# fritzsedlazeck/Sniffles

Hardware: AMD Instinct MI355X
Metric: SV-signatures clustered/sec (clustering + calling + QC + genotype + INS consensus) (higher is better)
Workload: dtype int32/f64

## Files before the change

### sniffles_amd/csrc/snf_fused.h

```cpp
#pragma once
#include "snf_stage_final.h"
#include "snf_stage_cluster.h"
#include "snf_stage_call.h"

namespace snf {

template <int K>
SNF_D void block_exscan256(const unsigned long long (&val)[K], unsigned long long (&excl)[K], unsigned long long (&tot)[K],
                           unsigned long long* lds) {
  const int tid = threadIdx.x, lane = tid & 63, wid = tid >> 6;
  unsigned long long incl[K];
#pragma unroll
  for (int k = 0; k < K; k++) {
    unsigned long long x = val[k];
#pragma unroll
    for (int d = 1; d < 64; d <<= 1) { const unsigned long long y = __shfl_up(x, d, 64); if (lane >= d) x += y; }
    incl[k] = x;
    if (lane == 63) lds[wid * K + k] = x;
  }
  __syncthreads();
#pragma unroll
  for (int k = 0; k < K; k++) {
    unsigned long long base = 0, all = 0;
#pragma unroll
// ... 93 lines not shown
          }
        }
        const unsigned long long inc = __ballot(state == 2);
        const int first = __ffsll((long long)inc) - 1;
        unsigned long long part = (inc == 0 || lane <= first) ? w : 0ull;
#pragma unroll
        for (int d = 32; d >= 1; d >>= 1) part += __shfl_xor(part, d, 64);
        ex += part;
        if (inc) done = true; else j -= 64;
      }
      if (lane == 0) { st_agent_u64(&st[2 * tile + 1], tagI | (ex + tot[k])); lds[k] = ex; }
    }
  }
  __syncthreads();
#pragma unroll
  for (int k = 0; k < K; k++) { off[k] = lds[k] + excl[k]; total[k] = lds[k] + tot[k]; }
  __syncthreads();
}
#define SNF_CHAIN_HEAD(name, slot)                                            \
  __global__ void __launch_bounds__(256) name(const View v, int64_t n) {      \
    __shared__ unsigned long long lds[24];                                    \
    const int64_t tile = chain_ticket(v, slot, lds);                          \
    const int64_t p = tile * 256 + threadIdx.x;


#define SNF_FUSED_HEAD(name)                                                  \
  __global__ void __launch_bounds__(256) name(const View v, int64_t n) {      \
    __shared__ unsigned long long lds[8];                                     \
    const int64_t p = (int64_t)blockIdx.x * 256 + threadIdx.x;

__global__ void __launch_bounds__(256) z0_init(const View v, int64_t n) {
  const int64_t i = (int64_t)blockIdx.x * 256 + threadIdx.x;
  const int64_t T = v.T, G = 8 * T + 8;
  if (i < (int64_t)(sizeof(Counts) / 8)) ((unsigned long long*)v.cnt)[i] = 0;
  if (i <= T) { v.t_cov_sum[i] = 0; v.t_status[i] = 0; }
  if (i <= T + 1) v.t_call_off[i] = 0;
  if (i < G) { v.grp_first_bin[i] = -1; v.grp_seed_lo[i] = -1; v.grp_seed_hi[i] = -1; v.grp_dirty[i] = 0; }
  if (i < TS_SLOTS * v.super_stride) v.tile_super[i] = 0;
  if (i < v.tile_stride) {
    v.tile_sums[(int64_t)TS_REFINED * v.tile_stride + i] = 0; v.tile_sums[(int64_t)TS_CALLS * v.tile_stride + i] = 0;
  }
  if (i == 0) *v.chain_epoch += 1u;
  if (v.wave_path && i < 3 * 64 * 16) v.big_cnt[i] = 0;
  if (v.wave_path && i < 3 * 64 * 16) v.d2cnt[i] = 0;
  if (i == 0 && v.NS > 0) {
    const int64_t N = v.NS;
    v.headflag[N] = 0; v.eligflag[N] = 0; v.fN[N] = 0; v.fL[N] = 0; v.runflag[N] = 0; v.clflag[N] = 0; v.rcflag[N] = 0; v.cdflag[N] = 0;
  }
}

SNF_FUSED_HEAD(a0k_keep)
  if (p < n) a0_keep_body(p, v);
  unsigned long long val[1] = {p < n ? (unsigned long long)v.pf_keep[p] : 0ull};
  tile_publish<1>(v, TS_KEEP, val, lds);
}
SNF_FUSED_HEAD(a0k_compact)
  unsigned long long val[1] = {p < n ? (unsigned long long)v.pf_keep[p] : 0ull}, off[1];
  tile_scan<1>(v, TS_KEEP, val, off, lds);
  if (p < n) {
    v.pf_scan[p] = (uint32_t)off[0];
    if (p == n - 1) v.cnt->n_kept = (int64_t)(off[0] + val[0]);
    a0_emit(p, v);
  }
}
SNF_FUSED_HEAD(a2k_heads)
  if (p < n) { a2_heads_body(p, v); v.rcflag[p] = 0; }
  unsigned long long val[1] = {p < n ? (unsigned long long)v.headflag[p] : 0ull};
// ... 201 lines not shown
```

### sniffles_amd/csrc/snf_lib.hip

```cpp
#include "snf_stage_final.h"
#include "snf_wave_refine.h"
#include "snf_wave_cons.h"
#include "snf_fused.h"
#include "snf_stage_window.h"
#include "snf_stage_out.h"
#include "snf_wave_call.h"
#include "snf_wave_call_g.h"
#include "snf_wave_refine_g.h"
#include "snf_ctx.h"

#include <rocprim/device/device_radix_sort.hpp>
#include <rocprim/device/device_scan.hpp>

#include <fcntl.h>
#include <sys/file.h>
#include <unistd.h>

#include <atomic>
#include <map>
#include <tuple>
#include <cmath>
#include <ctime>
#include <memory>
#include <mutex>
// ... 608 lines not shown
    so[i] = sl >= 0 ? t.seq_off[i] + p0 : 0;
  }
}
void stage_pool(const snf_task_input_t& t, uint8_t* st, size_t pool_at, int64_t p0, int64_t b0, int64_t b1, std::atomic<int>* has_dash) {
  if (memchr(t.seq_pool + b0, '-', (size_t)(b1 - b0))) has_dash->store(1);
  memcpy(st + pool_at + (size_t)(p0 + b0), t.seq_pool + b0, (size_t)(b1 - b0));
}
void stage_reads(const snf_task_input_t& t, uint8_t* st, const size_t* off, int64_t r0, int32_t* rend_max) {
  const int64_t r = t.n_reads;
  int32_t* rs = (int32_t*)(st + off[IC_RSTART]) + r0; int32_t* re = (int32_t*)(st + off[IC_REND]) + r0;
  uint8_t* rh = st + off[IC_RHP] + r0;
  bool sorted = true;
  for (int64_t i = 1; i < r; i++) if (t.read_start[i] < t.read_start[i - 1]) { sorted = false; break; }
  if (sorted) {
    if (r) { memcpy(rs, t.read_start, (size_t)r * 4); memcpy(re, t.read_end, (size_t)r * 4); memcpy(rh, t.read_hp, (size_t)r); }
  } else {
    std::vector<int64_t> ord((size_t)r);
    for (int64_t i = 0; i < r; i++) ord[(size_t)i] = i;
    std::stable_sort(ord.begin(), ord.end(), [&](int64_t x, int64_t y) { return t.read_start[x] < t.read_start[y]; });
    for (int64_t i = 0; i < r; i++) { const int64_t k = ord[(size_t)i]; rs[i] = t.read_start[k]; re[i] = t.read_end[k]; rh[i] = t.read_hp[k]; }
  }
  int32_t rmax = 0;
  for (int64_t i = 0; i < r; i++) {
    const int32_t s = rs[i], e = re[i];
    if (s < 0 || s >= t.contig_len || e < s) fail("read interval outside the task region (leadprov.py:497-498)");
    if (rh[i] > 2) fail("read hp must be 0, 1 or 2");
    if (e > rmax) rmax = e;
  }
  *rend_max = rmax;
}

void enqueue_read_index(snf_batch_impl* b);
void enqueue_pass_init(snf_batch_impl* b);
void join_open_candidates(snf_batch_impl* b);
void enqueue_keys(snf_batch_impl* b);
bool coverage_per_call(const snf_batch_impl* b) { return b->k.d4_thread || !b->v.wave_path; }

void do_upload(snf_batch_impl* b) {
  SNF_TRACE("snf_batch_upload");
  View& v = b->v;
  const double t_begin = now_ms();
  int T = (int)b->tasks.size();
  int64_t N = b->h_lead_off.back(), R = b->h_read_off.back(), NTR = (int64_t)b->h_trs.size();
  if (T >= (1 << 16)) fail("too many tasks in one batch (max 65535)");
  if (N >= (int64_t)1 << 31 || R >= (int64_t)1 << 31) fail("batch too large for 32-bit lead/read indices");
  v.cfg = b->cfg; v.T = T; v.N = N; v.R = R; v.NTR = NTR;
  const int gap_base = b->cfg.cluster_merge_bnd > (int)b->cfg.cluster_repeat_h_max ? b->cfg.cluster_merge_bnd : (int)b->cfg.cluster_repeat_h_max;
  v.run_gap = b->k.run_gap != KNOB_UNSET ? b->k.run_gap : (gap_base > 1000 ? gap_base : 1000);
  v.wave_path = b->k.wave_path ? 1 : 0;
  b->fused = b->k.fuse && N <= ((int64_t)1 << 25);
  v.prof = b->k.prof ? 1 : 0;
  v.merge_reread = b->k.merge_reread ? 1 : 0;
  {
    int64_t max_bins = 1;
    for (auto& t : b->tasks) { int64_t nb = t.contig_len / (b->cfg.cluster_binsize > 0 ? b->cfg.cluster_binsize : 1) + 1; if (nb > max_bins) max_bins = nb; }
    v.key_bin_bits = bits_for((uint64_t)max_bins);
    v.key_nbits = v.key_bin_bits + bits_for((uint64_t)(8 * (T > 0 ? T : 1)));
    v.key32 = (!b->k.sort64 && v.key_nbits + 1 <= 32) ? 1 : 0;
  }
  v.pool_len = b->h_pool_off.back(); v.pool_cap = 2 * v.pool_len + 16;
  v.pool_extra_base = v.pool_len; v.pool_slice = 0;
  if (b->slots_d1w > 0 && b->k.pool_slices) {
    v.pool_slice = (v.pool_len / b->slots_d1w) & ~(int64_t)15;
    v.pool_extra_base = v.pool_len + v.pool_slice * b->slots_d1w;
    v.pool_cap = v.pool_extra_base + v.pool_len + 16;
  }
// ... 172 lines not shown
  size_t N1 = (size_t)N + 1;
  v.key_in = dalloc<uint64_t>(b, N); v.key_out = dalloc<uint64_t>(b, N); v.val_in = dalloc<uint32_t>(b, N); v.val_out = dalloc<uint32_t>(b, N);
  {
    v.NS = N; v.prefilter = 0;
    std::vector<int64_t> cell_off((size_t)T + 1, 0);
    const int bs = b->cfg.cluster_binsize > 0 ? b->cfg.cluster_binsize : 1;
    for (int t = 0; t < T; t++) cell_off[(size_t)t + 1] = cell_off[(size_t)t] + (int64_t)SNF_NTYPES * ((int64_t)b->tasks[(size_t)t].contig_len / bs + 1);
    const int64_t cells = cell_off[(size_t)T];
    if (N > 0 && b->cfg.dev_min_leads_cluster >= 2 && b->k.prefilter && cells < ((int64_t)1 << 36)) {
      v.prefilter = 1;
      v.t_cell_off = upload_vec(b, cell_off);
      b->pf_words = (((cells >> 19) + 1) << 19) / 16 + 2;
      v.pf_spread = b->k.pf_spread ? 1 : 0;
      v.pf_bm = dalloc<uint32_t>(b, (size_t)b->pf_words);
      dzero(b, v.pf_bm, (size_t)b->pf_words * 4);
      v.pf_key = dalloc<uint64_t>(b, N); v.pf_keep = dalloc<uint32_t>(b, N1); v.pf_scan = dalloc<uint32_t>(b, N1);
      dsync(b);
    }
  }
  const int WIN_W_MAX = b->k.win_bits_max, WIN_W_MIN = 6;
  auto win_layout = [&](int W, std::vector<int64_t>& off) {
    const int bs = b->cfg.cluster_binsize > 0 ? b->cfg.cluster_binsize : 1;
    off.assign((size_t)T + 1, 0);
    for (int t = 0; t < T; t++) off[(size_t)t + 1] = off[(size_t)t] + (int64_t)SNF_NTYPES * ((((int64_t)b->tasks[(size_t)t].contig_len / bs + 1) >> W) + 1);
    return off[(size_t)T];
  };
  int64_t win_slots_max = 0;
  const bool front_wanted = v.prefilter && v.wave_path && b->k.winfront && b->k.fuse && N <= ((int64_t)1 << 25) && T < (1 << 17);
  if (front_wanted) {
    std::vector<int64_t> off;
    win_slots_max = win_layout(WIN_W_MIN, off);
    if (win_slots_max >= ((int64_t)1 << 31)) win_slots_max = 0;
  }
  v.front = 0; v.NW = 0;
  if (win_slots_max > 0) {
    const size_t W1 = (size_t)win_slots_max + 1;
    v.wcnt = dalloc<uint32_t>(b, W1); v.wfill = dalloc<uint32_t>(b, W1); v.wbase = dalloc<uint32_t>(b, W1);
    const size_t occ_max = (size_t)(N < win_slots_max ? N : win_slots_max) + 2;
    const size_t nblk = (size_t)N / 64 + 2;
    v.wlist = dalloc<uint32_t>(b, 4 * occ_max); v.blk_k0 = dalloc<uint32_t>(b, nblk);
    v.ws_seeds = dalloc<uint32_t>(b, nblk); v.ws_nf = dalloc<uint32_t>(b, nblk); v.ws_nl = dalloc<uint32_t>(b, nblk);
    v.whead = dalloc<uint64_t>(b, N1); v.whead2 = dalloc<uint64_t>(b, N1);
    dzero(b, v.wcnt, W1 * 4); dzero(b, v.wfill, W1 * 4);
  }
  uint32_t** u32s[] = {&v.headflag, &v.headscan, &v.eligflag, &v.eligscan, &v.fN, &v.pN, &v.fL, &v.pL, &v.runflag, &v.runscan,
                       &v.clflag, &v.clscan, &v.rcflag, &v.rcscan, &v.cdflag, &v.cdscan, &v.rnf, &v.rnp};
  for (auto pp : u32s) *pp = dalloc<uint32_t>(b, N1);
  v.seqnull = dalloc<uint8_t>(b, N); v.bin_lo = dalloc<int32_t>(b, N1); v.bin_key = dalloc<uint64_t>(b, N);
  v.bin_hap = dalloc<uint16_t>(b, 3 * (size_t)N); v.bin_elig = dalloc<uint8_t>(b, N);
  v.grp_first_bin = dalloc<int32_t>(b, 8 * (size_t)T + 8);
  v.L = dalloc<uint32_t>(b, N); v.LL = dalloc<uint32_t>(b, N); v.Lrec = dalloc<LeadRec>(b, N1); v.chdr = dalloc<ClusterHdr>(b, N1);
  int32_t** i32s[] = {&v.seed_bin, &v.seed_lo, &v.seed_hi, &v.seedL_lo, &v.seedL_hi, &v.seed_start, &v.seed_grp, &v.c_last, &v.c_end,
                      &v.nxt, &v.prv, &v.run_first, &v.run_last_head, &v.cl_head, &v.w0, &v.w1, &v.w2, &v.w3, &v.w4, &v.w5, &v.w6, &v.w7,
                      &v.F_orig, &v.F_svlen, &v.F_seq_len, &v.FI, &v.F_lpos, &v.rc_n_s, &v.rc_cl_s, &v.rc_lo, &v.rc_n, &v.rc_cluster};
  for (auto pp : i32s) *pp = dalloc<int32_t>(b, N1);
  double** f64s[] = {&v.s_mean0, &v.s_stdev0, &v.c_mean, &v.c_stdev, &v.run_b_stdev, &v.run_b_absmean};
  for (auto pp : f64s) *pp = dalloc<double>(b, N1);
  uint8_t** u8s[] = {&v.s_repeat0, &v.c_repeat, &v.run_b_repeat, &v.F_sel, &v.rc_keeplong_s, &v.rc_keeplong};
  for (auto pp : u8s) *pp = dalloc<uint8_t>(b, N1);
  v.c_ms = dalloc<ClusterSums>(b, N1);
  v.grp_dirty = dalloc<int32_t>(b, 8 * (size_t)T + 8); v.grp_seed_lo = dalloc<int32_t>(b, 8 * (size_t)T + 8);
  v.grp_seed_hi = dalloc<int32_t>(b, 8 * (size_t)T + 8);
  v.F_seq_off = dalloc<int64_t>(b, N1);
  v.fcopy = dalloc<FuseDesc>(b, N1); dzero(b, v.fcopy, N1 * sizeof(FuseDesc));
  v.cand = dalloc<snf_call_t>(b, N1); v.candx = dalloc<CallX>(b, N1);
  v.calls = dalloc<snf_call_t>(b, N1); v.callx = dalloc<CallX>(b, N1);
  v.rnames = dalloc<uint32_t>(b, 2 * (size_t)N + 1);
// ... 18 lines not shown
  { const int eb = b->k.e1_batch; v.e1_batch = (eb == 2 || eb == 4 || eb == 8 || eb == 16 || eb == 32) ? eb : 64; }
  v.stage_cap = b->k.big_stage ? 1 : 0;
  v.cdesc = dalloc<ConsDesc>(b, N1); v.crl_off = dalloc<int64_t>(b, N1); v.crl_len = dalloc<int32_t>(b, N1); v.aln_kept_w = dalloc<uint8_t>(b, N1);
  for (int k = 0; k < 8; k++) v.cls_list[k] = k == 6 ? nullptr : dalloc<int32_t>(b, N1);
  v.d2cap = (int64_t)(N1 / 64 + 64);
  for (int k = 0; k < 3; k++) v.d2_list[k] = dalloc<int32_t>(b, (size_t)(64 * v.d2cap));
  v.d2cnt = dalloc<uint32_t>(b, 3 * 64 * 16);
  v.d2_from_list = 0; v.d1_from_list = 0;
#ifdef SNF_ITRACE
  if (!v.itrace) { SNF_HIP(hipMalloc((void**)&v.itrace, (size_t)SNF_IT_SLOTS * SNF_IT_CAP * 8)); SNF_HIP(hipMemset(v.itrace, 0, (size_t)SNF_IT_SLOTS * SNF_IT_CAP * 8)); }
#endif
#ifdef SNF_WG_TRACE
  if (!v.wgtrace) { SNF_HIP(hipMalloc((void**)&v.wgtrace, (size_t)(1 << 20) * 24)); SNF_HIP(hipMemset(v.wgtrace, 0, (size_t)(1 << 20) * 24)); }
#endif
  v.cons_tab_off = dalloc<int64_t>(b, N1 + 1); v.cons_aln_off = dalloc<int64_t>(b, N1 + 1); v.cons_read_off = dalloc<int64_t>(b, N1 + 1);
  v.cons_tab_sz = dalloc<int64_t>(b, N1 + 1);
  v.sz_tab = dalloc<int64_t>(b, N1 + 1); v.sz_aln = dalloc<int64_t>(b, N1 + 1); v.sz_rd = dalloc<int64_t>(b, N1 + 1);
  v.sc_tab = dalloc<int64_t>(b, N1 + 1); v.sc_aln = dalloc<int64_t>(b, N1 + 1); v.sc_rd = dalloc<int64_t>(b, N1 + 1);
  const double t_alloc = now_ms();
  if (v.prefilter) {
    const bool tm = b->timing; b->timing = false;
    enqueue_pass_init(b);
    enqueue_keys(b);
    b->timing = tm;
    Counts hc{};
    d2h(b, &hc, v.cnt, sizeof(Counts));
    dsync(b);
    v.NS = hc.n_kept;
    if (v.prof) fprintf(stderr, "[SNF_PROF] prefilter: %lld of %lld leads share their (svtype, bin) cell with another lead\n", (long long)v.NS, (long long)N);
  }
  const double t_pfcount = now_ms();
  if (win_slots_max > 0 && v.NS > 0) {
    int forced = b->k.win_bits;
    int best_w = -1; int64_t best_occ = 0, best_max = 0, best_big = 0;
    std::vector<int64_t> off;
    if (forced && (forced < WIN_W_MIN || forced > WIN_W_MAX)) forced = 0;
    for (int W = forced ? forced : WIN_W_MAX; W >= (forced ? forced : WIN_W_MIN); W--) {
      v.NW = win_layout(W, off); v.win_bits = W;
      const int64_t* d_off = upload_vec(b, off);
      v.t_win_off = d_off;
      const bool tm = b->timing; b->timing = false;
      enqueue_pass_init(b);
      LAUNCH_Q(w1_hist, v, N, 0);
      LAUNCH_Q(w0_stats, v, v.NW, 0);
      b->timing = tm;
      Counts hc{};
      d2h(b, &hc, v.cnt, sizeof(Counts));
      dzero(b, v.wcnt, ((size_t)v.NW + 1) * 4);
      dsync(b);
      if (hc.max_win <= 256 || (best_w < 0 && hc.max_win <= SNF_WIN_MAXCAP)) { best_w = W; best_occ = hc.n_occ; best_max = hc.max_win; best_big = hc.n_big64; }
      if (hc.max_win <= 256) break;
    }
    if (best_w >= 0) {
      if (v.win_bits != best_w) { v.NW = win_layout(best_w, off); v.win_bits = best_w; v.t_win_off = upload_vec(b, off); dsync(b); }
      v.front = 1; b->h_n_occ = best_occ; b->win_cap = best_max <= 64 ? 64 : best_max <= 256 ? 256 : SNF_WIN_MAXCAP;
      b->h_n_big64 = best_big; v.w4_list = dalloc<int32_t>(b, (size_t)best_big + 64); v.w4_mode = 0;
    }
    if (v.prof) fprintf(stderr, "[SNF_PROF] window front end: %s (W = %d: %lld windows, %lld occupied, largest %lld leads, %lld of more than 64: w4s_segment in %s)\n", v.front ? "on" : "off",
                        v.win_bits, (long long)v.NW, (long long)best_occ, (long long)best_max, (long long)best_big,
                        (b->k.w4_split && b->win_cap > 64 && best_big > 0 && best_big * 8 < (N + 63) / 64) ? "two launches" : "one launch");
  }
  const double t_winsel = now_ms();
  {
    v.alt_cap = v.pool_cap; v.alt_pool = dalloc<uint8_t>(b, (size_t)v.alt_cap + 32);
    const size_t NO = (size_t)v.NS + 1;
    v.o_scan = dalloc<uint32_t>(b, N1 + 1); v.o_src = dalloc<int32_t>(b, N1); v.o_dst = dalloc<int32_t>(b, N1); v.o_key = dalloc<int32_t>(b, N1);
    v.o_rn = dalloc<int64_t>(b, N1);
    v.out_hdr = dalloc<OutHdr>(b, 1);
    dzero(b, v.out_hdr, sizeof(OutHdr));
    v.out_dev_cap = (int64_t)(NO * sizeof(snf_call_t) + (2 * (size_t)N + 1) * 4 + 1024);
    v.out_dev = dalloc<uint8_t>(b, (size_t)v.out_dev_cap);
    v.out_mode = b->out_mode; v.out_valid = 0; v.out_pin = nullptr; v.out_pin_cap = 0; v.alt_pin = nullptr; v.alt_pin_cap = 0;
  }
  const double t_index0 = now_ms();
  { const bool tm = b->timing; b->timing = false; enqueue_read_index(b); b->timing = tm; }
  {
    bool any_deep = false;
    for (int t = 0; t < T; t++) any_deep |= b->tasks[(size_t)t].n_reads >= 65536;
    std::vector<int32_t> maxd((size_t)T, 0);
    if (any_deep && R > 0) {
      MaxDepth md{v.r_start, v.re_sorted, v.rs_top, v.re_top, v.r_task, v.t_read_off, b->d_max_depth};
      const bool tm = b->timing; b->timing = false;
      LAUNCH_Q(r3_maxdepth, md, R, R * 8);
      b->timing = tm;
      d2h(b, maxd.data(), b->d_max_depth, sizeof(int32_t) * (size_t)T);
      dsync(b);
    }
    b->h_cov_exact.assign((size_t)T, 0);
    bool any = false;
    for (int t = 0; t < T; t++) {
// ... 145 lines not shown
    if (TS_SLOTS * v.super_stride > n0) n0 = TS_SLOTS * v.super_stride;
    if ((int64_t)(sizeof(Counts) / 8) > n0) n0 = (int64_t)(sizeof(Counts) / 8);
    if (3 * 64 * 16 > n0) n0 = 3 * 64 * 16;
    if (v.tile_stride > n0) n0 = v.tile_stride;
    FUSED(z0_init, n0);
  } else {
    dzero(b, v.cnt, sizeof(Counts));
    dzero(b, v.t_cov_sum, sizeof(unsigned long long) * (T + 1));
    dzero(b, v.t_status, sizeof(int32_t) * (T + 1));
    dzero(b, v.t_call_off, sizeof(int64_t) * (T + 2));
    dzero(b, v.grp_first_bin, sizeof(int32_t) * (8 * T + 8), 0xff);
    dzero(b, v.grp_seed_lo, sizeof(int32_t) * (8 * T + 8), 0xff);
    dzero(b, v.grp_seed_hi, sizeof(int32_t) * (8 * T + 8), 0xff);
    dzero(b, v.grp_dirty, sizeof(int32_t) * (8 * T + 8));
  }
}
void enqueue_keys(snf_batch_impl* b) {
  SNF_TRACE("A0: keys + occupancy prefilter");
  View& v = b->v;
  const int64_t N = v.N;
  if (N <= 0) return;
  LAUNCH(a1_keys, v, N, N * 21);
  if (!v.prefilter) return;
  if (b->fused) {
    { Scope _s(b, "a0_keep", N * 8); FUSED(a0k_keep, N); }
    FUSED(a0k_compact, N);
  } else {
    LAUNCH(a0_keep, v, N, N * 8);
    prim_exscan<uint32_t>(b, v.pf_keep, v.pf_scan, N + 1, "scan_keep");
    LAUNCH_Q(a0_compact, v, N, N * 12);
  }
}

void enqueue_window_front(snf_batch_impl* b) {
  SNF_TRACE("A: window front end");
  View& v = b->v;
  const int64_t N = v.N, NW = v.NW, n_occ = b->h_n_occ;
  if (N <= 0 || n_occ <= 0) return;
  Scope _all(b, "front_window", N * 21);
  LAUNCH_Q(w1_hist, v, N, 0);
  if (v.chain_on) CHAIN(w2c_offsets, NW);
  else { FUSED(w2a_sums, NW); FUSED(w2b_offsets, NW); }
  LAUNCH_Q(w3_scatter, v, N, 0);
  const int64_t n_blk = (N + 63) / 64;
  const bool split = b->k.w4_split && b->win_cap > 64 && b->h_n_big64 > 0 && b->h_n_big64 * 8 < n_blk;
  {
    Scope* sc = b->time_all ? new Scope(b, "w4s_segment", 0) : nullptr;
    if (split) {
      v.w4_mode = 1;
      hipLaunchKernelGGL(w4s_segment<64>, dim3((unsigned)n_blk), dim3(64), 0, b->cur, v, (int64_t)0);
      v.w4_mode = 2;
      if (b->win_cap == 256) hipLaunchKernelGGL(w4s_segment<256>, dim3((unsigned)b->h_n_big64), dim3(64), 0, b->cur, v, (int64_t)0);
      else hipLaunchKernelGGL(w4s_segment<SNF_WIN_MAXCAP>, dim3((unsigned)b->h_n_big64), dim3(64), 0, b->cur, v, (int64_t)0);
      v.w4_mode = 0;
    }
    else if (b->win_cap == 64) hipLaunchKernelGGL(w4s_segment<64>, dim3((unsigned)n_blk), dim3(64), 0, b->cur, v, (int64_t)0);
    else if (b->win_cap == 256) hipLaunchKernelGGL(w4s_segment<256>, dim3((unsigned)n_blk), dim3(64), 0, b->cur, v, (int64_t)0);
    else hipLaunchKernelGGL(w4s_segment<SNF_WIN_MAXCAP>, dim3((unsigned)n_blk), dim3(64), 0, b->cur, v, (int64_t)0);
    delete sc;
    SNF_HIP(hipGetLastError());
  }
  if (v.chain_on) CHAIN(w5c_offsets, n_blk);
  else { FUSED(w5a_sums, n_blk); FUSED(w5b_offsets, n_blk); }
  LAUNCH_Q(w6t_emit, v, N, 0);
}

void enqueue_fuse_copy(snf_batch_impl* b, hipEvent_t after) {
  View& v = b->v;
  if (!after) { SNF_HIP(hipEventRecord(b->ev_refined, b->stream)); after = b->ev_refined; }
  SNF_HIP(hipStreamWaitEvent(b->stream2, after, 0));
  hipStream_t prev = b->cur; b->cur = b->stream2;
  { Scope _s(b, "d1c_fusecopy", 0);
    int64_t grid = (v.NS + 63) / 64; if (grid > 2048) grid = 2048;
    hipLaunchKernelGGL(d1c_fusecopy, dim3((unsigned)grid), dim3(64), 0, b->cur, v, (int64_t)0);
    SNF_HIP(hipGetLastError()); }
  b->cur = prev;
// ... 653 lines not shown
    if (strcmp(t.name, "e1w_finalize") == 0) t.bytes = (int64_t)sizeof(snf_call_t) * b->h_cnt->n_calls;
    if (strcmp(t.name, "d4_coverage") == 0) t.bytes = 8 * b->v.R + 20 * b->h_cnt->n_calls;
    if (strcmp(t.name, "f4_emit") == 0 && b->v.res_out) t.bytes = 2 * ((int64_t)sizeof(snf_call_t) * b->v.res_out->n_out + 4 * b->v.res_out->rn_out);
  }
  for (const auto& t : b->timings) {
    bool found = false;
    for (auto& a : b->timing_acc)
      if (strcmp(a.name, t.name) == 0) { a.ms += t.ms; a.bytes = t.bytes; a.launches++; found = true; break; }
    if (!found) b->timing_acc.push_back({t.name, t.ms, t.bytes, 1});
  }
}

bool settle_alt_stage(snf_batch_impl* b) {
  View& v = b->v;
  if (!v.wave_path || !b->fused || v.NS <= 0) return false;
  const Counts& c = *b->h_cnt;
  if (c.n_cls[7] == 0 && c.n_cons_fallback == 0) return false;
  run_alt_fallback(b);
  LAUNCH_Q(z1_results, v, tail_threads(v), 0);
  dsync(b);
  return true;
}

void do_fetch(snf_batch_impl* b, int stage, snf_result_t* out) {
  SNF_TRACE(stage >= 1 ? "snf_batch_fetch(1): wait + result block" : "snf_batch_fetch(0): wait + candidates");
  View& v = b->v;
  int T = v.T;
  b->r_status.assign(T, 0); b->r_off.assign(T + 1, 0); b->r_cov.assign(T, NAN);
  full_sync(b);
  pass_waited(b);
  if (b->h_cnt->overflow) fail(b->h_cnt->overflow & 2 ? "internal: hand-over list of the call kernels overflowed" : "internal: fused-sequence pool overflow");
  if (v.prof) {
    const Counts& c = *b->h_cnt;
    fprintf(stderr, "[SNF_PROF] counts: valid %lld bins %lld seeds %lld clusters %lld refined %lld calls %lld | cons calls %lld reads %lld "
                    "fallback %lld alt bytes %lld fused bytes through the shared counter %llu (the rest in the waves' own slices; the split depends on scheduling, the total and the capacity do not) | ALT lists copy %llu small %llu large %llu/%llu/%llu/%llu thread %llu rows %llu\n", (long long)c.n_valid, (long long)c.n_bins, (long long)c.n_seeds, (long long)c.n_clusters,
            (long long)c.n_rc, (long long)c.n_calls, (long long)c.n_cons, (long long)c.n_cons_reads, (long long)c.n_cons_fallback,
            (long long)c.alt_total, c.pool_extra_used, c.n_cls[0], c.n_cls[1], c.n_cls[2], c.n_cls[3], c.n_cls[4], c.n_cls[5], c.n_cls[6], c.n_cls[7]);
  }
  memcpy(b->r_status.data(), v.res_status, (size_t)T * sizeof(int32_t));
  memcpy(b->r_cov.data(), v.res_cov, (size_t)T * sizeof(double));
  if (stage >= 1 && b->finalized) {
    const bool alt_late = settle_alt_stage(b);
    {
      const Counts& c = *b->h_cnt;
      bool skipped_work = false;
      for (int k = 0; k < 3; k++) {
        if (b->skipped_big[k] && c.n_big[k] > 0) skipped_work = true;
        b->hist_big[k] = c.n_big[k];
      }
      if (skipped_work) { b->pass_idle = true; fail("internal: a pass skipped x_big although items were handed to it (the handle's next pass launches it)"); }
      b->have_big_hist = true;
      b->hist_small = (int64_t)c.n_cls[1]; b->hist_large = (int64_t)(c.n_cls[2] + c.n_cls[3] + c.n_cls[4] + c.n_cls[5]); b->hist_copy = (int64_t)c.n_cls[0];
      b->hist_calls = c.n_calls; b->have_hist = true;
    }
    const OutHdr h = *v.res_out;
    const uint8_t* base = (const uint8_t*)b->hb_out.p;
    const int64_t alt_total_now = b->h_cnt->alt_total;
    const bool block_there = !h.in_pinned && b->staged_kernel && b->stage_block_copied && v.stage_out_pin == (uint8_t*)b->hb_out.p && h.bytes <= v.stage_out_cap;
    const bool alt_there = !b->h_cnt->alt_in_pinned && b->staged_kernel && b->stage_alt_copied && !alt_late && v.stage_alt_pin == (uint8_t*)b->hb_alt.p && alt_total_now <= v.stage_alt_cap;
    bool need_sync = false;
    std::unique_lock<std::mutex> copy_turn(pacing_of(b).copy_mu, std::defer_lock);
    if (b->staged && pace_copy_turn() && ((!h.in_pinned && !block_there) || (!b->h_cnt->alt_in_pinned && !alt_there))) copy_turn.lock();
    if (!h.in_pinned && !block_there) {
      v.out_pin = nullptr; v.out_pin_cap = 0;
      base = (const uint8_t*)b->hb_out.ensure((size_t)h.bytes + 256);
      d2h_timed(b, (void*)base, v.out_dev, (size_t)h.bytes, "d2h_block");
      need_sync = true;
    }
// ... 270 lines not shown
  const auto& lut = build_gt_lut(*cfg);
  DevArena& A = g_geno_arenas[device];
  std::lock_guard<std::mutex> hold(A.mu);
  ArenaLayout L;
  const size_t o_lut = L.add<GtEntry>(lut.size()), o_calls = L.add<snf_call_t>((size_t)n);
  if (!A.ensure(device, L.at)) fail("no HIP device available: the sniffles_amd hot path requires an AMD GPU (there is no CPU fallback)");
  memcpy(A.h + o_lut, lut.data(), lut.size() * sizeof(GtEntry));
  memcpy(A.h + o_calls, calls, (size_t)n * sizeof(snf_call_t));
  GenoView q{};
  q.cfg = *cfg; q.gt_lut = (const GtEntry*)(A.d + o_lut); q.calls = (snf_call_t*)(A.d + o_calls); q.n = n;
  SNF_HIP(hipMemcpyAsync(A.d, A.h, L.at, hipMemcpyHostToDevice, A.stream));
  hipLaunchKernelGGL(g1_genotype, dim3((unsigned)((n + 255) / 256)), dim3(256), 0, A.stream, q, n);
  SNF_HIP(hipGetLastError());
  SNF_HIP(hipMemcpyAsync(A.h + o_calls, A.d + o_calls, (size_t)n * sizeof(snf_call_t), hipMemcpyDeviceToHost, A.stream));
  SNF_HIP(hipStreamSynchronize(A.stream));
  memcpy(calls, A.h + o_calls, (size_t)n * sizeof(snf_call_t));
}
}

template <class T>
std::vector<T> pull(snf_batch_impl* b, const T* dptr, size_t n) {
  std::vector<T> h(n ? n : 1);
  d2h(b, h.data(), dptr, n * sizeof(T));
  return h;
}
void do_fetch_clusters(snf_batch_impl* b, int stage, snf_clusters_t* out) {
  View& v = b->v;
  if (stage < 0 || stage > 2) fail("stage must be 0 (seeds), 1 (merged) or 2 (refined)");
  if (!b->cov_avg_ready) fail("snf_batch_fetch_clusters needs snf_batch_call_candidates first");
  if (v.prefilter) {
    const bool fin = b->finalized;
    full_sync(b);
    v.prefilter = 0; v.front = 0; v.NS = v.N;
    run_call_candidates(b);
    if (fin) run_finalize(b);
  }
  full_sync(b);
  const Counts c = *b->h_cnt;
  b->cl_task.clear(); b->cl_svtype.clear(); b->cl_start.clear(); b->cl_end.clear(); b->cl_seed.clear(); b->cl_seed_index.clear();
  b->cl_nlong.clear(); b->cl_lead.clear(); b->cl_lead_svlen.clear(); b->cl_repeat.clear(); b->cl_lead_off.assign(1, 0);
  const int64_t N = v.N;
  if (N > 0 && c.n_seeds > 0) {
    const size_t ns = (size_t)c.n_seeds, ncl = (size_t)c.n_clusters, nrc = (size_t)c.n_rc, nf = (size_t)c.NF;
    auto seed_grp = pull(b, v.seed_grp, ns); auto seed_start = pull(b, v.seed_start, ns); auto seed_bin = pull(b, v.seed_bin, ns);
    auto seed_lo = pull(b, v.seed_lo, ns); auto seed_hi = pull(b, v.seed_hi, ns);
    auto seedL_lo = pull(b, v.seedL_lo, ns); auto seedL_hi = pull(b, v.seedL_hi, ns);
    auto s_repeat0 = pull(b, v.s_repeat0, ns);
    auto grp_first_bin = pull(b, v.grp_first_bin, (size_t)(8 * v.T + 8));
    auto L = pull(b, v.L, nf);
    auto lead_off = pull(b, v.t_lead_off, (size_t)v.T + 1);
    auto in_svlen = pull(b, v.in_svlen, (size_t)N);
    std::vector<int32_t> cl_head, c_last, c_end, rc_lo, rc_n, rc_cluster, FI, F_orig, F_svlen; std::vector<uint8_t> c_repeat, rc_keeplong;
    if (stage >= 1) { cl_head = pull(b, v.cl_head, ncl); c_last = pull(b, v.c_last, ns); c_end = pull(b, v.c_end, ns); c_repeat = pull(b, v.c_repeat, ns); }
    if (stage == 2) {
      rc_lo = pull(b, v.rc_lo, nrc); rc_n = pull(b, v.rc_n, nrc); rc_cluster = pull(b, v.rc_cluster, nrc); rc_keeplong = pull(b, v.rc_keeplong, nrc);
      FI = pull(b, v.FI, nf); F_orig = pull(b, v.F_orig, nf); F_svlen = pull(b, v.F_svlen, nf);
    }
    dsync(b);
    auto head = [&](int32_t h, int32_t last, int32_t end, uint8_t rep, int64_t nlong) {
      const int g = seed_grp[(size_t)h];
      b->cl_task.push_back(g >> 3); b->cl_svtype.push_back(g & 7); b->cl_start.push_back(seed_start[(size_t)h]); b->cl_end.push_back(end);
      b->cl_seed.push_back(seed_start[(size_t)h]); b->cl_seed_index.push_back(seed_bin[(size_t)h] - grp_first_bin[(size_t)g]);
      b->cl_nlong.push_back((int32_t)nlong); b->cl_repeat.push_back(rep);
      (void)last;
    };
    auto add_row = [&](uint32_t orig, int32_t svlen, int task) {
// ... 460 lines not shown
```

### sniffles_amd/csrc/snf_stage_window.h

```cpp
#pragma once
#include "snf_fused.h"
#include "snf_wave_refine.h"

namespace snf {

#define SNF_WIN_MAXCAP 1024

SNF_HD uint32_t win_pack(const View& v, uint32_t bin_low, bool is_long, uint32_t hap) { return bin_low | ((is_long ? 1u : 0u) << 12) | (hap << 13); }
SNF_HD uint32_t win_bin_low(uint32_t a) { return a & 0xfffu; }
SNF_HD bool win_is_long(uint32_t a) { return (a >> 12) & 1u; }
SNF_HD uint32_t win_hap(uint32_t a) { return (a >> 13) & 3u; }
SNF_D bool win_of_lead(const View& v, int64_t i, uint32_t* w, uint32_t* attr) {
  const int t = v.lead_task[i];
  const int64_t rs = v.in_ref_start[i];
  if (rs < 0 || rs >= v.t_contig_len[t]) return false;
  const uint64_t bin = (uint64_t)(rs / v.cfg.cluster_binsize);
  const int svtype = v.in_svtype[i];
  const int64_t w0 = v.t_win_off[t], nwin = (v.t_win_off[t + 1] - w0) / SNF_NTYPES;
  *w = (uint32_t)(w0 + (int64_t)svtype * nwin + (int64_t)(bin >> v.win_bits));
  *attr = win_pack(v, (uint32_t)(bin & ((1u << v.win_bits) - 1u)), svtype == SNF_INS && v.in_svlen[i] == SNF_SVLEN_NONE, v.in_hap[i]);
  return true;
}

SNF_D int win_group(bool valid, uint32_t w, int* count, bool* leader) {
  const int lane = threadIdx.x & 63;
  unsigned long long todo = __ballot(valid);
  int rank = 0, cnt = 0; bool lead = false;
  while (todo) {
    const int l0 = __ffsll((long long)todo) - 1;
    const uint32_t w0 = (uint32_t)__shfl((int)w, l0, 64);
    const unsigned long long same = __ballot(valid && w == w0);
    if (valid && w == w0) { cnt = __popcll(same); rank = __popcll(same & ((1ull << lane) - 1ull)); lead = lane == l0; }
    todo &= ~same;
  }
  *count = cnt; *leader = lead;
  return rank;
}

__global__ void __launch_bounds__(256) w1_hist(const View v, int64_t n) {
  IT_SCOPE(0)
  const int64_t i = (int64_t)blockIdx.x * 256 + threadIdx.x;
  uint32_t w = ~0u, attr = 0;
  const bool valid = i < n && win_of_lead(v, i, &w, &attr);
  if (i < n) { v.val_in[i] = valid ? w : ~0u; v.val_out[i] = attr; }
  if (i <= v.NS) v.rcflag[i] = 0;
  int cnt; bool leader;
  win_group(valid, w, &cnt, &leader);
  if (leader) atomicAdd(&v.wcnt[w], (uint32_t)cnt);
}

__global__ void __launch_bounds__(256) w0_stats(const View v, int64_t n) {
  const int64_t p = (int64_t)blockIdx.x * 256 + threadIdx.x;
  const uint32_t c = p < n ? v.wcnt[p] : 0u;
  const unsigned long long occ = __ballot(c != 0);
  uint32_t m = c;
#pragma unroll
  for (int d = 32; d >= 1; d >>= 1) { const uint32_t y = (uint32_t)__shfl_xor((int)m, d, 64); if (y > m) m = y; }
  const unsigned long long big = __ballot(c > 64u);
  if ((threadIdx.x & 63) == 0 && occ) {
    atomicAdd((unsigned long long*)&v.cnt->n_occ, (unsigned long long)__popcll(occ));
    atomicMax((unsigned long long*)&v.cnt->max_win, (unsigned long long)m);
    if (big) atomicAdd((unsigned long long*)&v.cnt->n_big64, (unsigned long long)__popcll(big));
  }
}

SNF_D void win_list(const View& v, int64_t p, uint32_t c, unsigned long long off, unsigned long long k) {
  if (p == 0) v.blk_k0[0] = 0;
  if (!c) return;
  int lo = 0, hi = v.T;
  while (hi - lo > 1) { const int mid = (lo + hi) >> 1; if (v.t_win_off[mid] <= p) lo = mid; else hi = mid; }
  ((uint4*)v.wlist)[k] = make_uint4((uint32_t)p, c, (uint32_t)off, (uint32_t)lo);
  for (unsigned long long bb = off / 64 + 1; bb <= (off + c) / 64; bb++) v.blk_k0[bb] = (uint32_t)(k + 1);
}

SNF_FUSED_HEAD(w2a_sums)
  const uint32_t c = p < n ? v.wcnt[p] : 0u;
  unsigned long long val[2] = {(unsigned long long)c, c ? 1ull : 0ull};
  tile_publish<2>(v, TS_WIN, val, lds);
}
SNF_FUSED_HEAD(w2b_offsets)
  const uint32_t c = p < n ? v.wcnt[p] : 0u;
  unsigned long long val[2] = {(unsigned long long)c, c ? 1ull : 0ull}, off[2];
  tile_scan<2>(v, TS_WIN, val, off, lds);
  if (p < n) {
    v.wcnt[p] = 0; v.wfill[p] = 0;
    v.wbase[p] = (uint32_t)off[0];
    win_list(v, p, c, off[0], off[1]);
    if (p == n - 1) { v.wbase[n] = (uint32_t)(off[0] + val[0]); v.cnt->n_valid = (int64_t)(off[0] + val[0]); v.cnt->n_occ = (int64_t)(off[1] + val[1]); }
  }
}

SNF_CHAIN_HEAD(w2c_offsets, TS_WIN)
  const uint32_t c = p < n ? v.wcnt[p] : 0u;
  unsigned long long val[2] = {(unsigned long long)c, c ? 1ull : 0ull}, off[2], tot[2];
  chain_scan<2>(v, TS_WIN, tile, val, off, tot, lds);
  if (p < n) {
    v.wcnt[p] = 0; v.wfill[p] = 0;
    v.wbase[p] = (uint32_t)off[0];
    win_list(v, p, c, off[0], off[1]);
    if (p == n - 1) { v.wbase[n] = (uint32_t)tot[0]; v.cnt->n_valid = (int64_t)tot[0]; v.cnt->n_occ = (int64_t)tot[1]; }
  }
}

__global__ void __launch_bounds__(256) w3_scatter(const View v, int64_t n) {
  IT_SCOPE(1)
  const int64_t i = (int64_t)blockIdx.x * 256 + threadIdx.x;
  const uint32_t w = i < n ? v.val_in[i] : ~0u;
  const bool valid = w != ~0u;
  int cnt; bool leader;
  const int rank = win_group(valid, w, &cnt, &leader);
  uint32_t first = 0;
  if (leader) first = atomicAdd(&v.wfill[w], (uint32_t)cnt);
  const int lane = threadIdx.x & 63;
  unsigned long long todo = __ballot(valid);
  uint32_t mine = 0;
  while (todo) {
    const int l0 = __ffsll((long long)todo) - 1;
    const uint32_t w0 = (uint32_t)__shfl((int)w, l0, 64);
    const uint32_t f0 = (uint32_t)__shfl((int)first, l0, 64);
    const unsigned long long same = __ballot(valid && w == w0);
    if (valid && w == w0) mine = f0;
    todo &= ~same;
  }
  (void)lane;
  if (valid) v.key_in[(int64_t)v.wbase[w] + mine + rank] = ((uint64_t)v.val_out[i] << 32) | (uint64_t)(uint32_t)i;
}

SNF_D int wave_runmax(int x, int carry) {
  x = wave_incl_max(x);
  return x > carry ? x : carry;
}

#define SNF_WS_NORM 1u
#define SNF_WS_LONG 2u
#define SNF_WS_SEQNULL 4u
#define SNF_WS_SEED 8u

SNF_D uint64_t wkey_make(uint32_t widx, uint64_t word) {
  const uint32_t a = (uint32_t)(word >> 32);
  return ((uint64_t)widx << 47) | ((uint64_t)win_bin_low(a) << 35) | ((uint64_t)(uint32_t)word << 3) | ((uint64_t)win_hap(a) << 1) | (win_is_long(a) ? 1ull : 0ull);
}
SNF_D uint32_t wkey_group(uint64_t k) { return (uint32_t)(k >> 35); }
SNF_D uint32_t wkey_bin(uint64_t k) { return (uint32_t)(k >> 35) & 0xfffu; }
SNF_D uint32_t wkey_widx(uint64_t k) { return (uint32_t)(k >> 47); }
SNF_D uint32_t wkey_index(uint64_t k) { return (uint32_t)(k >> 3); }
SNF_D bool wkey_long(uint64_t k) { return (k & 1ull) != 0; }
SNF_D uint32_t wkey_hap(uint64_t k) { return (uint32_t)(k >> 1) & 3u; }

template <int CAP>
__global__ void __launch_bounds__(64) w4s_segment(const View v, int64_t n_unused) {
  IT_SCOPE(2)
  constexpr int CAPW = CAP + 64, E = CAPW / 64, PAD = 8;
  __shared__ uint64_t keys[CAPW + CAP + PAD];
  __shared__ uint16_t widx[CAPW];
  uint16_t* const hpos = widx;
  __shared__ uint32_t sA[CAPW], sB[CAPW];
  __shared__ uint32_t wS[64], wG[64], wB[64];
  const int lane = threadIdx.x;
  int64_t i = blockIdx.x;
  if (v.w4_mode == 2) {
    if (i >= (int64_t)v.cnt->n_w4big) return;
    i = v.w4_list[i];
  }
  const int64_t B0 = 64 * i;
  const int64_t n_valid = v.cnt->n_valid;
  uint64_t w0 = 0;
  if (B0 + lane < n_valid) w0 = v.key_in[B0 + lane];
  uint32_t k0 = 0, k1 = 0;
  if (B0 < n_valid) { k0 = v.blk_k0[i]; k1 = B0 + 64 <= n_valid ? v.blk_k0[i + 1] : (uint32_t)v.cnt->n_occ; }
  const int nw = (int)(k1 - k0);
  if (nw <= 0) { if (lane == 0) { v.ws_seeds[i] = 0; v.ws_nf[i] = 0; v.ws_nl[i] = 0; } return; }
  uint4 wr = make_uint4(0, 0, 0, 0);
  if (lane < nw) wr = ((const uint4*)v.wlist)[k0 + lane];
  const int xlo = (int)((int64_t)(uint32_t)__builtin_amdgcn_readfirstlane((int)wr.z) - B0);
  const int xhi = (int)((int64_t)(uint32_t)__builtin_amdgcn_readlane((int)(wr.z + wr.y), nw - 1) - B0);
  if (v.w4_mode == 1 && __shfl(wave_incl_max(lane < nw ? (int)wr.y : 0), 63, 64) > CAP) {
    if (lane == 0) v.w4_list[atomicAdd(&v.cnt->n_w4big, 1ull)] = (int32_t)i;
    return;
  }
  uint64_t wd[E];
  wd[0] = w0;
#pragma unroll
  for (int j = 1; j < E; j++) { const int x = lane + 64 * j; wd[j] = x < xhi ? v.key_in[B0 + x] : 0ull; }
  if (lane < nw) {
    const int t = (int)wr.w;
    const int64_t o0 = v.t_win_off[t], nwin = (v.t_win_off[t + 1] - o0) / SNF_NTYPES, rem = (int64_t)wr.x - o0;
    wS[lane] = (uint32_t)((int64_t)wr.z - B0); wG[lane] = (uint32_t)(t * 8 + (int)(rem / nwin)); wB[lane] = (uint32_t)((rem % nwin) << v.win_bits);
  }
#pragma unroll
  for (int j = 0; j < E; j++) { const int x = lane + 64 * j; if (x < xhi) { sA[x] = 0; sB[x] = 0; widx[x] = 0; } }
  const int nall = __shfl(wave_incl_max(lane < nw ? (int)wr.y : 0), 63, 64);
  for (int p = lane; p < nall + PAD; p += 64) keys[xhi + p] = ~0ull;
  __syncthreads();
  if (lane < nw) widx[wS[lane]] = (uint16_t)(lane + 1);
  __syncthreads();
  uint64_t e[E];
  {
    int carry = 0;
#pragma unroll
    for (int j = 0; j < E; j++) {
      e[j] = 0;
      if (64 * j < xhi) {
// ... 104 lines not shown
  tile_publish<3>(v, TS_WINC, val, lds);
}
SNF_FUSED_HEAD(w5b_offsets)
  unsigned long long val[3] = {p < n ? (unsigned long long)v.ws_seeds[p] : 0ull, p < n ? (unsigned long long)v.ws_nf[p] : 0ull,
                               p < n ? (unsigned long long)v.ws_nl[p] : 0ull}, off[3];
  tile_scan<3>(v, TS_WINC, val, off, lds);
  if (p < n) {
    v.ws_seeds[p] = (uint32_t)off[0]; v.ws_nf[p] = (uint32_t)off[1]; v.ws_nl[p] = (uint32_t)off[2];
    if (p == n - 1) {
      const int64_t ns = (int64_t)(off[0] + val[0]);
      v.cnt->n_seeds = ns; v.cnt->n_bins = ns; v.cnt->NF = (int64_t)(off[1] + val[1]); v.cnt->NLL = (int64_t)(off[2] + val[2]);
      v.eligscan[v.NS] = (uint32_t)ns;
    }
  }
}

SNF_CHAIN_HEAD(w5c_offsets, TS_WINC)
  unsigned long long val[3] = {p < n ? (unsigned long long)v.ws_seeds[p] : 0ull, p < n ? (unsigned long long)v.ws_nf[p] : 0ull,
                               p < n ? (unsigned long long)v.ws_nl[p] : 0ull}, off[3], tot[3];
  chain_scan<3>(v, TS_WINC, tile, val, off, tot, lds);
  if (p < n) {
    v.ws_seeds[p] = (uint32_t)off[0]; v.ws_nf[p] = (uint32_t)off[1]; v.ws_nl[p] = (uint32_t)off[2];
    if (p == n - 1) {
      const int64_t ns = (int64_t)tot[0];
      v.cnt->n_seeds = ns; v.cnt->n_bins = ns; v.cnt->NF = (int64_t)tot[1]; v.cnt->NLL = (int64_t)tot[2];
      v.eligscan[v.NS] = (uint32_t)ns;
    }
  }
}

__global__ void __launch_bounds__(256) w6t_emit(const View v, int64_t n_unused) {
  IT_SCOPE(3)
  const int64_t p = (int64_t)blockIdx.x * 256 + threadIdx.x;
  if (p >= v.cnt->n_valid) return;
  const uint64_t word = v.key_out[p];
  const uint32_t hi = (uint32_t)(word >> 32), o = (uint32_t)word;
  if (!(hi & (SNF_WS_NORM | SNF_WS_LONG))) return;
  const int64_t owner = p / 64 - (int64_t)((hi >> 16) & 31u);
  const uint32_t rank = (hi >> 4) & 0xfffu;
  int64_t qf = 0, ql = 0;
  if (hi & SNF_WS_NORM) {
    qf = (int64_t)v.ws_nf[owner] + rank;
    v.L[qf] = o;
    const uint4* src = (const uint4*)&v.in_rec[o];
    uint4 q0 = src[0], q1 = src[1], q2 = src[2], q3 = src[3];
    static_assert(offsetof(LeadRec, seq_len) == 20 && offsetof(LeadRec, seq_off) == 24, "words of q1");
    if ((int32_t)q1.y >= 0 && (hi & SNF_WS_SEQNULL)) { q1.y = 0xffffffffu; q1.z = 0; q1.w = 0; }
    uint4* dst = (uint4*)&v.Lrec[qf];
    dst[0] = q0; dst[1] = q1; dst[2] = q2; dst[3] = q3;
  } else {
    ql = (int64_t)v.ws_nl[owner] + rank;
    v.LL[ql] = o;
  }
  if (hi & SNF_WS_SEED) {
    const uint64_t hd = v.whead[p], h2 = v.whead2[p];
    const uint32_t other = (uint32_t)(h2 >> 52);
    if (hi & SNF_WS_NORM) ql = (int64_t)v.ws_nl[owner] + other; else qf = (int64_t)v.ws_nf[owner] + other;
    const int64_t qs = (int64_t)v.ws_seeds[owner] + (hi >> 21);
    const int with_len = (int)(hd & 0xffffu), all = (int)((hd >> 16) & 0xffffu), h1 = (int)((hd >> 32) & 0xffffu), hh2 = (int)(hd >> 48);
    v.seed_bin[qs] = (int32_t)qs;
    v.seed_lo[qs] = (int32_t)qf; v.seed_hi[qs] = (int32_t)(qf + with_len);
    v.seedL_lo[qs] = (int32_t)ql; v.seedL_hi[qs] = (int32_t)(ql + all - with_len);
    v.seed_start[qs] = (int32_t)(uint32_t)h2;
    v.seed_grp[qs] = (int)((h2 >> 32) & 0xfffffu);
    v.bin_hap[3 * qs + 0] = (uint16_t)(all - h1 - hh2); v.bin_hap[3 * qs + 1] = (uint16_t)h1; v.bin_hap[3 * qs + 2] = (uint16_t)hh2;
  }
}
// ... 3 lines not shown
```

### sniffles_amd/csrc/snf_view.h

```cpp
#pragma once
#include "../../include/sniffles_amd.h"
#include "snf_rt.h"

namespace snf {

struct Counts {
  int64_t n_valid, n_bins, n_seeds, NF, NLL, n_runs, n_clusters, n_rc, n_calls;
  int64_t n_ins_calls, alt_total, n_cons, tab_total, aln_total, n_cons_reads, rn_total;
  int64_t n_dirty_groups;
  int64_t n_kept;
  int64_t n_big[3];
  int64_t n_occ;
  int64_t max_win;
  int64_t n_big64;
  unsigned long long n_w4big;
  int64_t n_cons_fallback;
  unsigned long long cons_bytes[4];
  unsigned long long n_cls[8];
  unsigned long long pool_extra_used;
#ifdef SNF_CONS_PROFILE
  unsigned long long dbg[32];
#endif
#ifdef SNF_C1_PROFILE
  unsigned long long c1p[16];
// ... 100 lines not shown
  const uint32_t *in_qname, *in_read_id;
  const int32_t *in_ps, *in_mate_contig, *in_mate_pos, *in_seq_len;
  const int64_t* in_seq_off;
  const double* in_nm;
  const uint8_t *in_svtype, *in_strand, *in_mapq, *in_source, *in_hap, *in_is_sa, *in_first, *in_rev;
  const int32_t* lead_task;
  uint8_t* pool;

  const int32_t* r_start; const int32_t* r_end; const uint8_t* r_hp; const int32_t* r_task;
  uint64_t *rk_in, *rk_out; uint32_t *rv_in, *rv_out;
  int32_t* re_sorted;
  int32_t *rs_top, *re_top;
  int32_t *rs_mid, *re_mid;
  uint64_t* pc_s2;
  uint64_t* pc_e2;
  uint32_t* rflag;

  const int32_t *nm_start, *nm_end;
  const int64_t* t_nm_off;
  const int32_t* t_cov_exact;

  const int32_t* tr_start; const int32_t* tr_end; const int32_t* tr_pmax;

  int32_t prefilter;
  int32_t pf_spread;
  uint32_t* pf_bm;
  const int64_t* t_cell_off;
  uint64_t* pf_key;
  uint32_t *pf_keep, *pf_scan;
  int32_t front;
  int32_t win_bits;
  int64_t NW;
  const int64_t* t_win_off;
  uint32_t *wcnt, *wfill;
  uint32_t* wbase;
  uint32_t* wlist;
  uint32_t* blk_k0;
  uint32_t *ws_seeds, *ws_nf, *ws_nl;
  uint64_t* whead;
  uint64_t* whead2;
  uint64_t *key_in, *key_out; uint32_t *val_in, *val_out;
  int key32, key_bin_bits, key_nbits;
  uint32_t *headflag, *headscan;
  uint32_t *eligflag, *eligscan;
  uint32_t *fN, *pN;
  uint32_t *fL, *pL;
  uint32_t *runflag, *runscan;
  uint32_t *clflag, *clscan;
  uint32_t *rcflag, *rcscan;
  uint32_t *cdflag, *cdscan;
  uint8_t* seqnull;
  int32_t* bin_lo;
  uint64_t* bin_key;
  uint16_t* bin_hap;
  uint8_t* bin_elig;
  int32_t* grp_first_bin;
  uint32_t* L;
  uint32_t* LL;
  LeadRec* Lrec;
  const LeadRec* in_rec;
  ClusterHdr* chdr;
  int32_t out_mode;
  int32_t out_valid;
  int32_t rn_defer;
  int32_t rn_from_src;
  uint32_t* o_scan;
// ... 90 lines not shown
```

Before: 3.487 billion.

## Build the window index once during upload and reuse it in every pass

During window-size selection the full window index (histogram, offsets, scatter) is now built at upload time. The stats reduction is folded into the offsets kernels, and the per-pass front end skips rebuilding the index when it is marked ready. The counts n_valid and n_occ are cached in the View and re-seeded into the counter at init. The rcflag clear moves from the histogram kernel to the emit kernel. This removes repeated hist/offsets/scatter launches per pass, in exchange for extra state and a fallback path when readprep_each_pass is set.

```diff
diff --git a/sniffles_amd/csrc/snf_fused.h b/sniffles_amd/csrc/snf_fused.h
--- a/sniffles_amd/csrc/snf_fused.h
+++ b/sniffles_amd/csrc/snf_fused.h
@@ -149,7 +149,12 @@
 __global__ void __launch_bounds__(256) z0_init(const View v, int64_t n) {
   const int64_t i = (int64_t)blockIdx.x * 256 + threadIdx.x;
   const int64_t T = v.T, G = 8 * T + 8;
-  if (i < (int64_t)(sizeof(Counts) / 8)) ((unsigned long long*)v.cnt)[i] = 0;
+  if (i < (int64_t)(sizeof(Counts) / 8)) {
+    unsigned long long c0 = 0;
+    if (v.win_ready && i == (int64_t)(offsetof(Counts, n_valid) / 8)) c0 = (unsigned long long)v.win_n_valid;
+    if (v.win_ready && i == (int64_t)(offsetof(Counts, n_occ) / 8)) c0 = (unsigned long long)v.win_n_occ;
+    ((unsigned long long*)v.cnt)[i] = c0;
+  }
   if (i <= T) { v.t_cov_sum[i] = 0; v.t_status[i] = 0; }
   if (i <= T + 1) v.t_call_off[i] = 0;
   if (i < G) { v.grp_first_bin[i] = -1; v.grp_seed_lo[i] = -1; v.grp_seed_hi[i] = -1; v.grp_dirty[i] = 0; }
diff --git a/sniffles_amd/csrc/snf_lib.hip b/sniffles_amd/csrc/snf_lib.hip
--- a/sniffles_amd/csrc/snf_lib.hip
+++ b/sniffles_amd/csrc/snf_lib.hip
@@ -664,6 +664,7 @@
 
 void enqueue_read_index(snf_batch_impl* b);
 void enqueue_pass_init(snf_batch_impl* b);
+void enqueue_window_index(snf_batch_impl* b, bool scatter);
 void join_open_candidates(snf_batch_impl* b);
 void enqueue_keys(snf_batch_impl* b);
 bool coverage_per_call(const snf_batch_impl* b) { return b->k.d4_thread || !b->v.wave_path; }
@@ -902,7 +903,7 @@
     win_slots_max = win_layout(WIN_W_MIN, off);
     if (win_slots_max >= ((int64_t)1 << 31)) win_slots_max = 0;
   }
-  v.front = 0; v.NW = 0;
+  v.front = 0; v.NW = 0; v.win_ready = 0; v.win_stats = 0; v.win_n_valid = 0; v.win_n_occ = 0;
   if (win_slots_max > 0) {
     const size_t W1 = (size_t)win_slots_max + 1;
     v.wcnt = dalloc<uint32_t>(b, W1); v.wfill = dalloc<uint32_t>(b, W1); v.wbase = dalloc<uint32_t>(b, W1);
@@ -987,30 +988,35 @@
   const double t_pfcount = now_ms();
   if (win_slots_max > 0 && v.NS > 0) {
     int forced = b->k.win_bits;
-    int best_w = -1; int64_t best_occ = 0, best_max = 0, best_big = 0;
+    int best_w = -1; Counts best{};
     std::vector<int64_t> off;
     if (forced && (forced < WIN_W_MIN || forced > WIN_W_MAX)) forced = 0;
-    for (int W = forced ? forced : WIN_W_MAX; W >= (forced ? forced : WIN_W_MIN); W--) {
+    const bool tm = b->timing; b->timing = false;
+    auto count_windows = [&](int W) {
       v.NW = win_layout(W, off); v.win_bits = W;
-      const int64_t* d_off = upload_vec(b, off);
-      v.t_win_off = d_off;
-      const bool tm = b->timing; b->timing = false;
+      v.t_win_off = upload_vec(b, off);
       enqueue_pass_init(b);
-      LAUNCH_Q(w1_hist, v, N, 0);
-      LAUNCH_Q(w0_stats, v, v.NW, 0);
-      b->timing = tm;
+      v.win_stats = 1; enqueue_window_index(b, false); v.win_stats = 0;
       Counts hc{};
       d2h(b, &hc, v.cnt, sizeof(Counts));
-      dzero(b, v.wcnt, ((size_t)v.NW + 1) * 4);
       dsync(b);
-      if (hc.max_win <= 256 || (best_w < 0 && hc.max_win <= SNF_WIN_MAXCAP)) { best_w = W; best_occ = hc.n_occ; best_max = hc.max_win; best_big = hc.n_big64; }
+      return hc;
+    };
+    for (int W = forced ? forced : WIN_W_MAX; W >= (forced ? forced : WIN_W_MIN); W--) {
+      const Counts hc = count_windows(W);
+      if (hc.max_win <= 256 || (best_w < 0 && hc.max_win <= SNF_WIN_MAXCAP)) { best_w = W; best = hc; }
       if (hc.max_win <= 256) break;
     }
+    if (best_w >= 0 && v.win_bits != best_w) best = count_windows(best_w);
+    const int64_t best_occ = best.n_occ, best_max = best.max_win, best_big = best.n_big64;
     if (best_w >= 0) {
-      if (v.win_bits != best_w) { v.NW = win_layout(best_w, off); v.win_bits = best_w; v.t_win_off = upload_vec(b, off); dsync(b); }
+      LAUNCH_Q(w3_scatter, v, N, 0);
       v.front = 1; b->h_n_occ = best_occ; b->win_cap = best_max <= 64 ? 64 : best_max <= 256 ? 256 : SNF_WIN_MAXCAP;
+      v.win_n_valid = best.n_valid; v.win_n_occ = best_occ;
+      v.win_ready = b->k.readprep_each_pass ? 0 : 1;
       b->h_n_big64 = best_big; v.w4_list = dalloc<int32_t>(b, (size_t)best_big + 64); v.w4_mode = 0;
     }
+    b->timing = tm;
     if (v.prof) fprintf(stderr, "[SNF_PROF] window front end: %s (W = %d: %lld windows, %lld occupied, largest %lld leads, %lld of more than 64: w4s_segment in %s)\n", v.front ? "on" : "off",
                         v.win_bits, (long long)v.NW, (long long)best_occ, (long long)best_max, (long long)best_big,
                         (b->k.w4_split && b->win_cap > 64 && best_big > 0 && best_big * 8 < (N + 63) / 64) ? "two launches" : "one launch");
@@ -1222,16 +1228,22 @@
   }
 }
 
+void enqueue_window_index(snf_batch_impl* b, bool scatter) {
+  View& v = b->v;
+  const int64_t N = v.N, NW = v.NW;
+  LAUNCH_Q(w1_hist, v, N, 0);
+  if (v.chain_on) CHAIN(w2c_offsets, NW);
+  else { FUSED(w2a_sums, NW); FUSED(w2b_offsets, NW); }
+  if (scatter) LAUNCH_Q(w3_scatter, v, N, 0);
+}
+
 void enqueue_window_front(snf_batch_impl* b) {
   SNF_TRACE("A: window front end");
   View& v = b->v;
-  const int64_t N = v.N, NW = v.NW, n_occ = b->h_n_occ;
+  const int64_t N = v.N, n_occ = b->h_n_occ;
   if (N <= 0 || n_occ <= 0) return;
   Scope _all(b, "front_window", N * 21);
-  LAUNCH_Q(w1_hist, v, N, 0);
-  if (v.chain_on) CHAIN(w2c_offsets, NW);
-  else { FUSED(w2a_sums, NW); FUSED(w2b_offsets, NW); }
-  LAUNCH_Q(w3_scatter, v, N, 0);
+  if (!v.win_ready) enqueue_window_index(b, true);
   const int64_t n_blk = (N + 63) / 64;
   const bool split = b->k.w4_split && b->win_cap > 64 && b->h_n_big64 > 0 && b->h_n_big64 * 8 < n_blk;
   {
@@ -1951,8 +1963,8 @@
   if (b->h_cnt->overflow) fail(b->h_cnt->overflow & 2 ? "internal: hand-over list of the call kernels overflowed" : "internal: fused-sequence pool overflow");
   if (v.prof) {
     const Counts& c = *b->h_cnt;
-    fprintf(stderr, "[SNF_PROF] counts: valid %lld bins %lld seeds %lld clusters %lld refined %lld calls %lld | cons calls %lld reads %lld "
-                    "fallback %lld alt bytes %lld fused bytes through the shared counter %llu (the rest in the waves' own slices; the split depends on scheduling, the total and the capacity do not) | ALT lists copy %llu small %llu large %llu/%llu/%llu/%llu thread %llu rows %llu\n", (long long)c.n_valid, (long long)c.n_bins, (long long)c.n_seeds, (long long)c.n_clusters,
+    fprintf(stderr, "[SNF_PROF] counts: valid %lld windows %lld bins %lld seeds %lld clusters %lld refined %lld calls %lld | cons calls %lld reads %lld "
+                    "fallback %lld alt bytes %lld fused bytes through the shared counter %llu (the rest in the waves' own slices; the split depends on scheduling, the total and the capacity do not) | ALT lists copy %llu small %llu large %llu/%llu/%llu/%llu thread %llu rows %llu\n", (long long)c.n_valid, (long long)c.n_occ, (long long)c.n_bins, (long long)c.n_seeds, (long long)c.n_clusters,
             (long long)c.n_rc, (long long)c.n_calls, (long long)c.n_cons, (long long)c.n_cons_reads, (long long)c.n_cons_fallback,
             (long long)c.alt_total, c.pool_extra_used, c.n_cls[0], c.n_cls[1], c.n_cls[2], c.n_cls[3], c.n_cls[4], c.n_cls[5], c.n_cls[6], c.n_cls[7]);
   }
@@ -2289,6 +2301,7 @@
     const bool fin = b->finalized;
     full_sync(b);
     v.prefilter = 0; v.front = 0; v.NS = v.N;
+    v.win_ready = 0;
     run_call_candidates(b);
     if (fin) run_finalize(b);
   }
diff --git a/sniffles_amd/csrc/snf_stage_window.h b/sniffles_amd/csrc/snf_stage_window.h
--- a/sniffles_amd/csrc/snf_stage_window.h
+++ b/sniffles_amd/csrc/snf_stage_window.h
@@ -43,24 +43,24 @@
   uint32_t w = ~0u, attr = 0;
   const bool valid = i < n && win_of_lead(v, i, &w, &attr);
   if (i < n) { v.val_in[i] = valid ? w : ~0u; v.val_out[i] = attr; }
-  if (i <= v.NS) v.rcflag[i] = 0;
   int cnt; bool leader;
   win_group(valid, w, &cnt, &leader);
   if (leader) atomicAdd(&v.wcnt[w], (uint32_t)cnt);
 }
 
-__global__ void __launch_bounds__(256) w0_stats(const View v, int64_t n) {
-  const int64_t p = (int64_t)blockIdx.x * 256 + threadIdx.x;
-  const uint32_t c = p < n ? v.wcnt[p] : 0u;
-  const unsigned long long occ = __ballot(c != 0);
+SNF_D void win_stats(const View& v, uint32_t c) {
+  __shared__ uint32_t st_max[4], st_big[4];
   uint32_t m = c;
 #pragma unroll
   for (int d = 32; d >= 1; d >>= 1) { const uint32_t y = (uint32_t)__shfl_xor((int)m, d, 64); if (y > m) m = y; }
   const unsigned long long big = __ballot(c > 64u);
-  if ((threadIdx.x & 63) == 0 && occ) {
-    atomicAdd((unsigned long long*)&v.cnt->n_occ, (unsigned long long)__popcll(occ));
-    atomicMax((unsigned long long*)&v.cnt->max_win, (unsigned long long)m);
-    if (big) atomicAdd((unsigned long long*)&v.cnt->n_big64, (unsigned long long)__popcll(big));
+  if ((threadIdx.x & 63) == 0) { st_max[threadIdx.x >> 6] = m; st_big[threadIdx.x >> 6] = (uint32_t)__popcll(big); }
+  __syncthreads();
+  if (threadIdx.x == 0) {
+    uint32_t mm = st_max[0], nb = st_big[0];
+    for (int k = 1; k < 4; k++) { if (st_max[k] > mm) mm = st_max[k]; nb += st_big[k]; }
+    if (mm) atomicMax((unsigned long long*)&v.cnt->max_win, (unsigned long long)mm);
+    if (nb) atomicAdd((unsigned long long*)&v.cnt->n_big64, (unsigned long long)nb);
   }
 }
 
@@ -88,6 +88,7 @@
     win_list(v, p, c, off[0], off[1]);
     if (p == n - 1) { v.wbase[n] = (uint32_t)(off[0] + val[0]); v.cnt->n_valid = (int64_t)(off[0] + val[0]); v.cnt->n_occ = (int64_t)(off[1] + val[1]); }
   }
+  if (v.win_stats) win_stats(v, c);
 }
 
 SNF_CHAIN_HEAD(w2c_offsets, TS_WIN)
@@ -100,6 +101,7 @@
     win_list(v, p, c, off[0], off[1]);
     if (p == n - 1) { v.wbase[n] = (uint32_t)tot[0]; v.cnt->n_valid = (int64_t)tot[0]; v.cnt->n_occ = (int64_t)tot[1]; }
   }
+  if (v.win_stats) win_stats(v, c);
 }
 
 __global__ void __launch_bounds__(256) w3_scatter(const View v, int64_t n) {
@@ -163,11 +165,11 @@
     i = v.w4_list[i];
   }
   const int64_t B0 = 64 * i;
-  const int64_t n_valid = v.cnt->n_valid;
+  const int64_t n_valid = v.win_ready ? v.win_n_valid : v.cnt->n_valid;
   uint64_t w0 = 0;
   if (B0 + lane < n_valid) w0 = v.key_in[B0 + lane];
   uint32_t k0 = 0, k1 = 0;
-  if (B0 < n_valid) { k0 = v.blk_k0[i]; k1 = B0 + 64 <= n_valid ? v.blk_k0[i + 1] : (uint32_t)v.cnt->n_occ; }
+  if (B0 < n_valid) { k0 = v.blk_k0[i]; k1 = B0 + 64 <= n_valid ? v.blk_k0[i + 1] : (uint32_t)(v.win_ready ? v.win_n_occ : v.cnt->n_occ); }
   const int nw = (int)(k1 - k0);
   if (nw <= 0) { if (lane == 0) { v.ws_seeds[i] = 0; v.ws_nf[i] = 0; v.ws_nl[i] = 0; } return; }
   uint4 wr = make_uint4(0, 0, 0, 0);
@@ -338,7 +340,8 @@
 __global__ void __launch_bounds__(256) w6t_emit(const View v, int64_t n_unused) {
   IT_SCOPE(3)
   const int64_t p = (int64_t)blockIdx.x * 256 + threadIdx.x;
-  if (p >= v.cnt->n_valid) return;
+  if (p <= v.NS) v.rcflag[p] = 0;
+  if (p >= (v.win_ready ? v.win_n_valid : v.cnt->n_valid)) return;
   const uint64_t word = v.key_out[p];
   const uint32_t hi = (uint32_t)(word >> 32), o = (uint32_t)word;
   if (!(hi & (SNF_WS_NORM | SNF_WS_LONG))) return;
diff --git a/sniffles_amd/csrc/snf_view.h b/sniffles_amd/csrc/snf_view.h
--- a/sniffles_amd/csrc/snf_view.h
+++ b/sniffles_amd/csrc/snf_view.h
@@ -156,6 +156,9 @@
   int32_t win_bits;
   int64_t NW;
   const int64_t* t_win_off;
+  int32_t win_ready;
+  int32_t win_stats;
+  int64_t win_n_valid, win_n_occ;
   uint32_t *wcnt, *wfill;
   uint32_t* wbase;
   uint32_t* wlist;
```

Measured after the change: 3.786 billion, median of 6. 1.09x the previous value.
